# HorizonRobotics/HoloAgent

Measured on AMD Instinct MI355X. Metric: HMSG frames/sec (one scene per GPU: map A1-A2, fusion A3-A5, merge A6, pooling A7, floors A8, rooms by the device watershed N1, room clouds, room embeddings and View nodes A9, objects with the view <-> object test A10 and graph assembly A11, nothing handed in -- plus 1000 coarse-to-fine retrieval qu, higher is better.
Workload: dtype f64 geometry / f32 features

## Files before the change

holoagent_amd/csrc/hmsg_map.hip:

```cpp
#include "hmsg_common.h"

#include <atomic>

#include <algorithm>


__global__ void k_scan_lookback(const unsigned* __restrict__ in, unsigned* __restrict__ out, size_t n,
                                unsigned long long* __restrict__ state, unsigned epoch) {
    __shared__ unsigned wsum[4];
    __shared__ unsigned s_prefix;
    const int tid = threadIdx.x, lane = tid & 63, w = tid >> 6;
    const long long tile = blockIdx.x;
    const size_t base = ((size_t)tile * 256 + tid) * 4;
    unsigned v[4];
    unsigned t = 0;
    for (int i = 0; i < 4; ++i) {
        v[i] = base + i < n ? in[base + i] : 0u;
        t += v[i];
    }
    unsigned incl = t;
    for (int o = 1; o < 64; o <<= 1) {
        unsigned u = __shfl_up(incl, o);
        if (lane >= o) incl += u;
    }
// ... 113 lines not shown
                pix_at(pw, d, f, x, y);
                double w[3];
                if ((unsigned)f == ff && backproject(depth[g], x, y, cam, scale, T, w[0], w[1], w[2])) {
                    for (int a = 0; a < 3; ++a) {
                        mn[a] = w[a] < mn[a] ? w[a] : mn[a];
                        mx[a] = w[a] > mx[a] ? w[a] : mx[a];
                    }
                    cnt++;
                }
            }
        }
    }
    for (int a = 0; a < 3; ++a) {
        mn[a] = wave_min_f64(mn[a]);
        mx[a] = wave_max_f64(mx[a]);
    }
    int c = wave_sum_i32((int)cnt);
    if ((threadIdx.x & 63) == 0) {
        for (int a = 0; a < 3; ++a) {
            atomicMin(&out[a], enc_f64(mn[a]));
            atomicMax(&out[3 + a], enc_f64(mx[a]));
        }
        atomicAdd(npts, (unsigned long long)c);
    }
}

__global__ void k_mark(const unsigned short* __restrict__ depth, const double* __restrict__ pose, CamK cam, float scale,
                       int H, int W, int F, GridGeom g, unsigned long long* __restrict__ bitmap) {
    const size_t HW = (size_t)H * W;
    const size_t total = HW * F;
    for (size_t c0 = (size_t)blockIdx.x * PIX_CHUNK; c0 < total; c0 += (size_t)gridDim.x * PIX_CHUNK) {
        const PixWalk pw = pix_walk(c0, HW, W);
        const unsigned npix = (unsigned)(total - c0 < (size_t)PIX_CHUNK ? total - c0 : (size_t)PIX_CHUNK);
        const unsigned fl = pix_last_frame(pw, npix);
        for (unsigned ff = pw.f0; ff <= fl; ++ff) {
            const double* const T = pose + (size_t)ff * 16;
            for (unsigned d = threadIdx.x; d < npix; d += blockDim.x) {
                const size_t i = c0 + d;
                int f, x, y;
                pix_at(pw, d, f, x, y);
                double wx, wy, wz;
                if ((unsigned)f != ff || !backproject(depth[i], x, y, cam, scale, T, wx, wy, wz)) continue;
                int ix, iy, iz;
                cell_of(g, wx, wy, wz, ix, iy, iz);
                long long lin = lin_of(g, ix, iy, iz);
                unsigned long long bit = 1ull << (lin & 63);
                unsigned long long* wp = bitmap + (lin >> 6);
                if (!(*wp & bit)) atomicOr(wp, bit);
            }
        }
    }
}

struct VoxAcc {
    unsigned long long* sr;
    unsigned long long* sg;
    unsigned long long* sb;
    unsigned* n;
};

#define RUN_CHUNK 4096
__device__ __forceinline__ unsigned pixel_slot(const unsigned short* __restrict__ depth, const double* __restrict__ T ,
                                               const CamK& cam, float scale, size_t i, int x, int y, const GridGeom& g,
                                               const unsigned long long* __restrict__ bitmap, const unsigned* __restrict__ rank) {
    double wx, wy, wz;
    if (!backproject(depth[i], x, y, cam, scale, T, wx, wy, wz)) return 0xffffffffu;
    int ix, iy, iz;
    cell_of(g, wx, wy, wz, ix, iy, iz);
    const long long lin = lin_of(g, ix, iy, iz);
    const unsigned long long word = bitmap[lin >> 6];
    return rank[lin >> 6] + (unsigned)__popcll(word & ((1ull << (lin & 63)) - 1ull));
}

__global__ void __launch_bounds__(256) k_slots(const unsigned short* __restrict__ depth, const unsigned char* __restrict__ rgb,
                                               const double* __restrict__ pose, CamK cam, float scale, int H, int W, int F,
                                               GridGeom g, const unsigned long long* __restrict__ bitmap,
                                               const unsigned* __restrict__ rank, VoxAcc acc, unsigned* __restrict__ slots,
                                               unsigned* __restrict__ chunk_runs) {
    __shared__ unsigned s_runs;
    if (threadIdx.x == 0) s_runs = 0u;
    __syncthreads();
    const size_t HW = (size_t)H * W;
    const size_t total = HW * F;
    const int lane = threadIdx.x & 63;
    unsigned myruns = 0;
    const PixWalk pw = pix_walk((size_t)blockIdx.x * RUN_CHUNK, HW, W);
    const size_t left = total - (size_t)blockIdx.x * RUN_CHUNK;
    const unsigned fl = pix_last_frame(pw, (unsigned)(left < (size_t)RUN_CHUNK ? left : (size_t)RUN_CHUNK));
    for (int it = 0; it < RUN_CHUNK / 256; ++it) {
        const size_t i = (size_t)blockIdx.x * RUN_CHUNK + (size_t)it * 256 + threadIdx.x;
        const bool in_range = i < total;
        unsigned slot = 0xffffffffu;
        unsigned cr = 0, cg = 0, cb = 0, cn = 0;
        int x = 0;
        if (in_range) {
            int f, y;
            pix_at(pw, (unsigned)it * 256u + threadIdx.x, f, x, y);
            for (unsigned ff = pw.f0; ff <= fl; ++ff)
                if ((unsigned)f == ff) slot = pixel_slot(depth, pose + (size_t)ff * 16, cam, scale, i, x, y, g, bitmap, rank);
            slots[i] = slot;
            if (slot != 0xffffffffu) {
                const unsigned char* c = rgb + i * 3;
                cr = c[0];
                cg = c[1];
                cb = c[2];
                cn = 1;
            }
        }
        const unsigned prev = __shfl_up(slot, 1);
        int flag = (lane == 0 || prev != slot || x == 0) ? 1 : 0;
        const int head = flag;
        for (int d = 1; d < 64; d <<= 1) {
            unsigned tr = __shfl_up(cr, d), tg = __shfl_up(cg, d), tb = __shfl_up(cb, d), tn = __shfl_up(cn, d);
            int tf = __shfl_up(flag, d);
            if (lane >= d && !flag) {
                cr += tr; cg += tg; cb += tb; cn += tn;
                flag = tf;
            }
        }
        const int nhead = __shfl_down(head, 1);
        const bool tail = lane == 63 || nhead != 0;
        if (tail && slot != 0xffffffffu) {
            atomicAdd(&acc.sr[slot], (unsigned long long)cr);
            atomicAdd(&acc.sg[slot], (unsigned long long)cg);
            atomicAdd(&acc.sb[slot], (unsigned long long)cb);
            atomicAdd(&acc.n[slot], cn);
            ++myruns;
        }
    }
    myruns = (unsigned)wave_sum_i32((int)myruns);
    if (lane == 0 && myruns) atomicAdd(&s_runs, myruns);
    __syncthreads();
    if (threadIdx.x == 0) chunk_runs[blockIdx.x] = s_runs;
}

__global__ void __launch_bounds__(256) k_emit_runs(const unsigned* __restrict__ slots, size_t total, int W, size_t HW,
                                                   const unsigned* __restrict__ chunk_base, unsigned* __restrict__ keys,
                                                   unsigned long long* __restrict__ vals) {
    __shared__ unsigned s_w[4];
    __shared__ unsigned s_run;
    if (threadIdx.x == 0) s_run = chunk_base[blockIdx.x];
    __syncthreads();
    const int lane = threadIdx.x & 63, w = threadIdx.x >> 6;
    const PixWalk pw = pix_walk((size_t)blockIdx.x * RUN_CHUNK, HW, W);
    for (int it = 0; it < RUN_CHUNK / 256; ++it) {
        const size_t i = (size_t)blockIdx.x * RUN_CHUNK + (size_t)it * 256 + threadIdx.x;
        const bool in_range = i < total;
        const unsigned slot = in_range ? slots[i] : 0xffffffffu;
        int pf = 0, x = 0, py = 0;
        if (in_range) pix_at(pw, (unsigned)it * 256u + threadIdx.x, pf, x, py);
        const unsigned prev = __shfl_up(slot, 1);
        const bool head = lane == 0 || prev != slot || x == 0;
        const unsigned long long heads = __ballot(head);
        const int nhead = __shfl_down(head ? 1 : 0, 1);
        const bool tail = (lane == 63 || nhead != 0) && slot != 0xffffffffu;
        const unsigned long long tails = __ballot(tail);
        if (lane == 0) s_w[w] = (unsigned)__popcll(tails);
        __syncthreads();
        unsigned base = s_run;
        for (int q = 0; q < w; ++q) base += s_w[q];
        if (tail) {
            const unsigned long long below = heads & ((lane == 63) ? ~0ull : ((1ull << (lane + 1)) - 1ull));
            const int start_lane = 63 - __clzll(below);
            const unsigned len = (unsigned)(lane - start_lane + 1);
            const unsigned pos = base + (unsigned)__popcll(tails & ((1ull << lane) - 1ull));
            keys[pos] = slot;
            vals[pos] = ((unsigned long long)(unsigned)pf << 32) | ((unsigned long long)(unsigned)py << 20) |
                        ((unsigned long long)(unsigned)(x - (lane - start_lane)) << 8) | (unsigned long long)len;
        }
        __syncthreads();
        if (threadIdx.x == 0) s_run += s_w[0] + s_w[1] + s_w[2] + s_w[3];
        __syncthreads();
    }
}

template <bool LDS_SUM>
__global__ void __launch_bounds__(256) k_accum_ordered(const unsigned short* __restrict__ depth, const double* __restrict__ pose,
                                                       CamK cam, float scale, int W, size_t HW, long long V,
                                                       const unsigned* __restrict__ off, const unsigned long long* __restrict__ runs,
                                                       const unsigned* __restrict__ cnt, double* __restrict__ pts) {
    __shared__ double s_pt[LDS_SUM ? 4 : 1][LDS_SUM ? 64 * 3 : 1];
    const int lane = threadIdx.x & 63;
    double* const my_pt = s_pt[LDS_SUM ? (threadIdx.x >> 6) : 0];
    const long long v = ((long long)blockIdx.x * blockDim.x + threadIdx.x) >> 6;
    if (v >= V) return;
    double sx = 0.0, sy = 0.0, sz = 0.0;
    const unsigned r0 = off[v], r1 = off[v + 1];
    for (unsigned rb = r0; rb < r1; rb += 64) {
        const unsigned long long myrec = rb + lane < r1 ? runs[rb + lane] : 0ull;
        const int mylen = (int)(myrec & 255ull);
        int incl = mylen;
        for (int o = 1; o < 64; o <<= 1) {
            const int u = __shfl_up(incl, o);
            if (lane >= o) incl += u;
        }
        const int nrun = (int)min(64u, r1 - rb);
        int q0 = 0;
        while (q0 < nrun) {
            const int base = q0 ? __shfl(incl, q0 - 1) : 0;
            const unsigned long long fits = __ballot(lane >= q0 && lane < nrun && incl - base <= 64);
            const int q1 = q0 + __popcll(fits);
            const int npix = __shfl(incl, q1 - 1) - base;
            double wx = 0.0, wy = 0.0, wz = 0.0;
            unsigned long long rec = 0ull;
            int start = 0;
            for (int q = q0; q < q1; ++q) {
                const unsigned long long rq = __shfl(myrec, q);
                const int eq = __shfl(incl, q) - base;
                const int sq = eq - (int)(rq & 255ull);
                if (lane >= sq && lane < eq) {
                    rec = rq;
                    start = sq;
                }
            }
            if (lane < npix) {
                const int f = (int)(rec >> 32);
                const int y = (int)((rec >> 20) & 0xfffull), x0 = (int)((rec >> 8) & 0xfffull);
                const int x = x0 + (lane - start);
                backproject(depth[(size_t)f * HW + (size_t)y * W + x], x, y, cam, scale, pose + (size_t)f * 16, wx, wy, wz);
            }
            if (LDS_SUM) {
                my_pt[lane * 3] = wx;
                my_pt[lane * 3 + 1] = wy;
                my_pt[lane * 3 + 2] = wz;
                __builtin_amdgcn_wave_barrier();
                if (lane < 3)
                    for (int j = 0; j < npix; ++j) sx = __dadd_rn(sx, my_pt[j * 3 + lane]);
                __builtin_amdgcn_wave_barrier();
            } else {
                for (int j = 0; j < npix; ++j) {
                    sx = __dadd_rn(sx, wave_bcast_f64(wx, j));
                    sy = __dadd_rn(sy, wave_bcast_f64(wy, j));
                    sz = __dadd_rn(sz, wave_bcast_f64(wz, j));
                }
            }
            q0 = q1;
        }
    }
    if (LDS_SUM) {
        if (lane < 3) pts[v * 3 + lane] = __ddiv_rn(sx, (double)cnt[v]);
    } else if (lane == 0) {
        const double n = (double)cnt[v];
        pts[v * 3 + 0] = __ddiv_rn(sx, n);
        pts[v * 3 + 1] = __ddiv_rn(sy, n);
        pts[v * 3 + 2] = __ddiv_rn(sz, n);
    }
}

__global__ void k_slot_cells(const unsigned long long* __restrict__ bitmap, const unsigned* __restrict__ rank,
                             GridGeom g, int* __restrict__ cell ) {
    long long w = (long long)blockIdx.x * blockDim.x + threadIdx.x;
    if (w >= g.nwords) return;
    unsigned long long bits = bitmap[w];
    unsigned s = rank[w];
    while (bits) {
        int b = __ffsll(bits) - 1;
        bits &= bits - 1;
        long long lin = w * 64 + b;
        int iz = (int)(lin % g.nzp);
        long long r = lin / g.nzp;
        int iy = (int)(r % g.ny);
        int ix = (int)(r / g.ny);
        cell[(size_t)s * 3 + 0] = ix;
        cell[(size_t)s * 3 + 1] = iy;
        cell[(size_t)s * 3 + 2] = iz;
        ++s;
    }
}

__global__ void k_finalize(VoxAcc acc, long long V, double* __restrict__ cols) {
    long long s = (long long)blockIdx.x * blockDim.x + threadIdx.x;
    if (s >= V) return;
    double n = (double)acc.n[s];
    cols[s * 3 + 0] = ((double)acc.sr[s] / 255.0) / n;
    cols[s * 3 + 1] = ((double)acc.sg[s] / 255.0) / n;
    cols[s * 3 + 2] = ((double)acc.sb[s] / 255.0) / n;
}

__device__ __forceinline__ unsigned long long bits_range(int lo, int hi) {
    if (hi < lo) return 0ull;
    unsigned long long m = (hi >= 63) ? ~0ull : ((1ull << (hi + 1)) - 1ull);
    return m & ~((1ull << lo) - 1ull);
}

__global__ void k_outlier(const double* __restrict__ pts, const int* __restrict__ cell, long long V, GridGeom g,
                          const unsigned long long* __restrict__ bitmap, const unsigned* __restrict__ rank,
                          double radius, int nb_points, unsigned* __restrict__ keep) {
    const int lane = threadIdx.x & 63;
    const long long s = ((long long)blockIdx.x * blockDim.x + threadIdx.x) >> 6;
    if (s >= V) return;
    const double px = pts[s * 3], py = pts[s * 3 + 1], pz = pts[s * 3 + 2];
    const int cx = cell[s * 3], cy = cell[s * 3 + 1];
    const int R = (int)ceil(radius / g.vs) + 1;
    const int side = 2 * R + 1;
    const double r2 = radius * radius;
    const double slack = 1e-7;
    int count = 0;
    for (int c = lane; c < side * side; c += 64) {
        int ix = cx - R + c / side, iy = cy - R + c % side;
        if (ix < 0 || iy < 0 || ix >= g.nx || iy >= g.ny) continue;
        double xlo = g.ox + ix * g.vs, xhi = xlo + g.vs, ylo = g.oy + iy * g.vs, yhi = ylo + g.vs;
        double dxmin = fmax(0.0, fmax(xlo - px, px - xhi)), dxmax = fmax(fabs(px - xlo), fabs(px - xhi));
        double dymin = fmax(0.0, fmax(ylo - py, py - yhi)), dymax = fmax(fabs(py - ylo), fabs(py - yhi));
        dxmin = fmax(0.0, dxmin - slack);
        dymin = fmax(0.0, dymin - slack);
        dxmax += slack;
        dymax += slack;
        double rem_out = r2 - (dxmin * dxmin + dymin * dymin);
        if (rem_out <= 0.0) continue;
        double ho = sqrt(rem_out) + slack;
        int zo0 = (int)floor((pz - ho - g.oz) / g.vs), zo1 = (int)floor((pz + ho - g.oz) / g.vs);
        zo0 = zo0 < 0 ? 0 : zo0;
        zo1 = zo1 >= g.nz ? g.nz - 1 : zo1;
        if (zo1 < zo0) continue;
        double rem_in = r2 - (dxmax * dxmax + dymax * dymax);
        int zi0 = 1, zi1 = 0;
        if (rem_in > 0.0) {
            double hi_ = sqrt(rem_in) - slack;
            if (hi_ > 0.0) {
                zi0 = (int)ceil((pz - hi_ - g.oz) / g.vs);
                zi1 = (int)floor((pz + hi_ - g.oz) / g.vs) - 1;
                zi0 = zi0 < zo0 ? zo0 : zi0;
                zi1 = zi1 > zo1 ? zo1 : zi1;
            }
        }
        long long colw = ((long long)ix * g.ny + iy) * (g.nzp >> 6);
        for (int w = zo0 >> 6; w <= zo1 >> 6; ++w) {
            unsigned long long word = bitmap[colw + w];
            if (!word) continue;
// ... 146 lines not shown
            });
    }
}

void hmsg_build_map(hmsg_ctx* h) {
    const hmsg_config& c = h->cfg;
    hipStream_t s = h->stream;
    HMSG_REQUIRE(h->n_frames > 0, HMSG_ERR_INVALID, "hmsg_finalize_map: no frames added");
    HMSG_REQUIRE(c.voxel_size >= 0.01, HMSG_ERR_UNSUPPORTED,
                 "voxel_size < 0.01: the DBSCAN(0.01,100) of graph.py:352 is no longer a provable no-op");
    const int H = c.height, W = c.width, F = h->n_frames;
    const float scale = (float)c.depth_scale;
    const size_t total = (size_t)H * W * F;
    const unsigned nblk = (unsigned)std::min<size_t>(cdiv(total, 256), 256 * 8);

    DevBuf<unsigned long long> d_b;
    d_b.alloc(8);
    unsigned long long init[8] = {~0ull, ~0ull, ~0ull, 0ull, 0ull, 0ull, 0ull, 0ull};
    HIP_TRY(hipMemcpyAsync(d_b.p, init, sizeof(init), hipMemcpyHostToDevice, s));
    hipLaunchKernelGGL(k_bounds, dim3(nblk), dim3(256), 0, s, (const unsigned short*)h->depth.p,
                       (const double*)h->pose.p, h->cam, scale, H, W, F, d_b.p, d_b.p + 6);
    HMSG_CHECK_LAUNCH();
    unsigned long long hb[8];
    HIP_TRY(hipMemcpyAsync(hb, d_b.p, sizeof(hb), hipMemcpyDeviceToHost, s));
    HIP_TRY(hipStreamSynchronize(s));
    HMSG_REQUIRE(hb[6] > 0, HMSG_ERR_INVALID, "no valid depth pixel in any frame");
    double mn[3], mx[3];
    for (int a = 0; a < 3; ++a) {
        mn[a] = dec_f64(hb[a]);
        mx[a] = dec_f64(hb[3 + a]);
    }
    GridGeom g;
    g.vs = c.voxel_size;
    g.ox = mn[0] - g.vs * 0.5;
    g.oy = mn[1] - g.vs * 0.5;
    g.oz = mn[2] - g.vs * 0.5;
    g.nx = (int)floor((mx[0] - g.ox) / g.vs) + 2;
    g.ny = (int)floor((mx[1] - g.oy) / g.vs) + 2;
    g.nz = (int)floor((mx[2] - g.oz) / g.vs) + 2;
    g.nzp = (g.nz + 63) / 64 * 64;
    g.nwords = (long long)g.nx * g.ny * (g.nzp / 64);
    HMSG_REQUIRE(g.nwords < (1ll << 31), HMSG_ERR_UNSUPPORTED, "scene bounding box too large for the dense occupancy bitmap");
    h->grid = g;

    h->bitmap.alloc((size_t)g.nwords);
    h->rank.alloc((size_t)g.nwords);
    h->bitmap.zero(s);
    hipLaunchKernelGGL(k_mark, dim3(nblk), dim3(256), 0, s, (const unsigned short*)h->depth.p, (const double*)h->pose.p,
                       h->cam, scale, H, W, F, g, h->bitmap.p);
    HMSG_CHECK_LAUNCH();
    unsigned long long V0 = hmsg_bitmap_rank(h->bitmap.p, h->rank.p, (size_t)g.nwords, s, h->scan_tmp);
    h->V0 = (long long)V0;

    DevBuf<unsigned long long> srgb;
    DevBuf<unsigned> sn, slots, chunk_runs;
    srgb.alloc(V0 * 3);
    sn.alloc(V0);
    srgb.zero(s);
    sn.zero(s);
    slots.alloc(total);
    const unsigned nchunks = cdiv(total, RUN_CHUNK);
    chunk_runs.alloc((size_t)nchunks + 1);
    VoxAcc acc{srgb.p, srgb.p + V0, srgb.p + 2 * V0, sn.p};
    {
        ProfScope ps(h->prof, s, "k_slots", (double)total * 9.0 + (double)V0 * 28.0);
        hipLaunchKernelGGL(k_slots, dim3(nchunks), dim3(256), 0, s, (const unsigned short*)h->depth.p,
                           (const unsigned char*)h->rgb.p, (const double*)h->pose.p, h->cam, scale, H, W, F, g,
                           (const unsigned long long*)h->bitmap.p, (const unsigned*)h->rank.p, acc, slots.p, chunk_runs.p);
    }
    HMSG_CHECK_LAUNCH();
    unsigned long long nruns = 0;
    hmsg_scan_u32(chunk_runs.p, chunk_runs.p, (size_t)nchunks, s, h->scan_tmp, &nruns);
    SortBufs sb;
    sb.keys.alloc((size_t)std::max<unsigned long long>(nruns, 1));
    sb.vals.alloc((size_t)std::max<unsigned long long>(nruns, 1));
    HMSG_REQUIRE(W < 4096 && H < 4096, HMSG_ERR_UNSUPPORTED, "image sides must be below 4096 pixels");
    hipLaunchKernelGGL(k_emit_runs, dim3(nchunks), dim3(256), 0, s, (const unsigned*)slots.p, total, W, (size_t)H * W,
                       (const unsigned*)chunk_runs.p, sb.keys.p, sb.vals.p);
    HMSG_CHECK_LAUNCH();
    {
        ProfScope ps(h->prof, s, "sort_runs", (double)nruns * 12.0 * 4.0);
        hmsg_sort_pairs(sb, (size_t)nruns, bits_for(V0), s);
    }
    DevBuf<unsigned> run_off;
    run_off.alloc(V0 + 1);
    hmsg_sort_segment_starts(sb.res_keys, (size_t)nruns, run_off.p, (unsigned)V0, s);
    DevBuf<int> cell;
    cell.alloc(V0 * 3);
    hipLaunchKernelGGL(k_slot_cells, dim3(cdiv((size_t)g.nwords, 256)), dim3(256), 0, s,
                       (const unsigned long long*)h->bitmap.p, (const unsigned*)h->rank.p, g, cell.p);
    HMSG_CHECK_LAUNCH();
    DevBuf<double> pts0, cols0;
    pts0.alloc(V0 * 3);
    cols0.alloc(V0 * 3);
    {
        static const bool lds_sum = getenv("HMSG_DEBUG_ACCUM_WAVES") == nullptr;
        ProfScope ps(h->prof, s, "k_accum_ordered", (double)total * 2.0 + (double)nruns * 8.0 + (double)V0 * 32.0);
        hipLaunchKernelGGL(lds_sum ? k_accum_ordered<true> : k_accum_ordered<false>, dim3(cdiv(V0 * 64, 256)), dim3(256), 0, s,
                           (const unsigned short*)h->depth.p, (const double*)h->pose.p, h->cam, scale, W, (size_t)H * W, (long long)V0,
                           (const unsigned*)run_off.p, (const unsigned long long*)sb.res_vals, (const unsigned*)sn.p, pts0.p);
        HMSG_CHECK_LAUNCH();
        if (getenv("HMSG_DEBUG_ACCUM_STATS")) {
            std::vector<unsigned> hc((size_t)V0);
            HIP_TRY(hipMemcpyAsync(hc.data(), sn.p, (size_t)V0 * 4, hipMemcpyDeviceToHost, s));
            HIP_TRY(hipStreamSynchronize(s));
            std::sort(hc.begin(), hc.end());
            double tot = 0;
            for (unsigned c : hc) tot += c;
            fprintf(stderr, "[hmsg map] voxels %lld  runs %llu  pixels %.0f  max %u  median %u  p99 %u\n", (long long)V0, nruns, tot, hc.back(),
                    hc[hc.size() / 2], hc[(size_t)(hc.size() * 0.99)]);
            for (unsigned th : {512u, 2048u, 8192u, 32768u, 131072u}) {
                double px = 0;
                long long nv = 0;
                for (unsigned c : hc)
                    if (c > th) px += c, ++nv;
                fprintf(stderr, "[hmsg map]   more than %6u pixels: %7lld voxels holding %.3f of the pixels\n", th, nv, px / tot);
            }
        }
    }
    hipLaunchKernelGGL(k_finalize, dim3(cdiv(V0, 256)), dim3(256), 0, s, acc, (long long)V0, cols0.p);
    HMSG_CHECK_LAUNCH();

    DevBuf<unsigned> keep, newidx;
    keep.alloc(V0);
    newidx.alloc(V0);
    hipLaunchKernelGGL(k_outlier, dim3(cdiv(V0 * 64, 256)), dim3(256), 0, s, (const double*)pts0.p, (const int*)cell.p,
                       (long long)V0, g, (const unsigned long long*)h->bitmap.p, (const unsigned*)h->rank.p,
                       c.outlier_radius, c.outlier_nb_points, keep.p);
    HMSG_CHECK_LAUNCH();
    unsigned long long V = 0;
    hmsg_scan_u32(keep.p, newidx.p, V0, s, h->scan_tmp, &V);
    h->V = (long long)V;
    h->pts.alloc(V * 3);
    h->cols.alloc(V * 3);
    hipLaunchKernelGGL(k_compact, dim3(cdiv(V0, 256)), dim3(256), 0, s, (const unsigned*)keep.p, (const unsigned*)newidx.p,
                       (long long)V0, (const double*)pts0.p, (const double*)cols0.p, (const int*)cell.p, g, h->pts.p,
                       h->cols.p, h->bitmap.p);
    HMSG_CHECK_LAUNCH();
    unsigned long long V2 = hmsg_bitmap_rank(h->bitmap.p, h->rank.p, (size_t)g.nwords, s, h->scan_tmp);
    HMSG_REQUIRE(V2 == V, HMSG_ERR_INVALID, "internal: filtered bitmap population mismatch");
    const long long VR = (long long)V0 - (long long)V;
    h->have_cand = false;
    if (VR > 0 && V > 0) {
        h->bitmap_rm.alloc((size_t)g.nwords);
        h->rank_rm.alloc((size_t)g.nwords);
        h->bitmap_rm.zero(s);
        DevBuf<int> rmcell, rend;
        DevBuf<double> ub2;
        DevBuf<unsigned> ccnt, cursor;
        rmcell.alloc((size_t)VR * 3);
        rend.alloc((size_t)VR);
        ub2.alloc((size_t)VR);
        ccnt.alloc((size_t)VR + 1);
        cursor.alloc((size_t)VR);
        ccnt.zero(s);
        cursor.zero(s);
        hipLaunchKernelGGL(k_rm_cells, dim3(cdiv(V0, 256)), dim3(256), 0, s, (const unsigned*)keep.p, (const unsigned*)newidx.p,
                           (long long)V0, (const int*)cell.p, g, rmcell.p, h->bitmap_rm.p);
        HMSG_CHECK_LAUNCH();
        unsigned long long nrm = hmsg_bitmap_rank(h->bitmap_rm.p, h->rank_rm.p, (size_t)g.nwords, s, h->scan_tmp);
        HMSG_REQUIRE((long long)nrm == VR, HMSG_ERR_INVALID, "internal: removed-cell bitmap population mismatch");
        h->cand_off.alloc((size_t)VR + 1);
        {
            ProfScope ps(h->prof, s, "k_cand");
            hipLaunchKernelGGL(k_cand, dim3(cdiv((size_t)VR * 64, 256)), dim3(256), 0, s, 0, (const int*)rmcell.p, VR, g,
                               (const unsigned long long*)h->bitmap.p, (const unsigned*)h->rank.p, (const double*)h->pts.p, ub2.p,
                               rend.p, ccnt.p, (const unsigned*)nullptr, (int*)nullptr, (unsigned*)nullptr);
        }
        HMSG_CHECK_LAUNCH();
        unsigned long long ncand = 0;
        hmsg_scan_u32(ccnt.p, h->cand_off.p, (size_t)VR + 1, s, h->scan_tmp, &ncand);
        h->cand.alloc((size_t)std::max<unsigned long long>(ncand, 1));
        hipLaunchKernelGGL(k_cand, dim3(cdiv((size_t)VR * 64, 256)), dim3(256), 0, s, 1, (const int*)rmcell.p, VR, g,
                           (const unsigned long long*)h->bitmap.p, (const unsigned*)h->rank.p, (const double*)h->pts.p, ub2.p,
// ... 9 lines not shown
```

holoagent_amd/csrc/hmsg_pool.hip:

```cpp
#include "hmsg_boundary.h"
#include "hmsg_cloudops.h"
#include "hmsg_nn.h"
#include "hmsg_dbscan.h"

#include <algorithm>
#include <cmath>

typedef float f32x16 __attribute__((ext_vector_type(16)));

__global__ void k_pool_nn(const double* __restrict__ q, long long N, NNIndex I, double max_dist, int* __restrict__ idx,
                          unsigned* __restrict__ valid, TieList ties) {
    long long i = (long long)blockIdx.x * blockDim.x + threadIdx.x;
    if (i >= N) return;
    double d2 = 0;
    int ntie = 0;
    int v = nn_search(I, q[i * 3], q[i * 3 + 1], q[i * 3 + 2], &d2, &ntie);
    if (ntie > 1) tie_push(ties, i, q[i * 3], q[i * 3 + 1], q[i * 3 + 2]);
    idx[i] = v;
    valid[i] = (v >= 0 && __dsqrt_rn(d2) <= max_dist) ? 1u : 0u;
}

__global__ void k_pool_gather(const int* __restrict__ idx, const unsigned* __restrict__ valid, const unsigned* __restrict__ pos,
                              long long N, const float* __restrict__ feats, int D, float* __restrict__ X, float* __restrict__ Xn) {
    const int lane = threadIdx.x & 63;
// ... 96 lines not shown
            const float a0 = sa[wr * 64 + (lane & 31)][kk], a1 = sa[wr * 64 + 32 + (lane & 31)][kk];
            const float b0 = sb[wc * 64 + (lane & 31)][kk], b1 = sb[wc * 64 + 32 + (lane & 31)][kk];
            acc[0][0] = __builtin_amdgcn_mfma_f32_32x32x2f32(a0, b0, acc[0][0], 0, 0, 0);
            acc[0][1] = __builtin_amdgcn_mfma_f32_32x32x2f32(a0, b1, acc[0][1], 0, 0, 0);
            acc[1][0] = __builtin_amdgcn_mfma_f32_32x32x2f32(a1, b0, acc[1][0], 0, 0, 0);
            acc[1][1] = __builtin_amdgcn_mfma_f32_32x32x2f32(a1, b1, acc[1][1], 0, 0, 0);
        }
        __syncthreads();
    }
    const bool diag_tile = (ti == tj);
    for (int si = 0; si < 2; ++si)
        for (int sj = 0; sj < 2; ++sj) {
            const int rbase = r0 + wr * 64 + si * 32, cbase = c0 + wc * 64 + sj * 32;
            const int col = cbase + (lane & 31);
            unsigned mirror = 0u;
            for (int r = 0; r < 16; ++r) {
                const int rloc = (r & 3) + 8 * (r >> 2) + 4 * (lane >> 5);
                const int row = rbase + rloc;
                float d = __fadd_rn(-acc[si][sj][r], 1.0f);
                d = fminf(fmaxf(d, 0.f), 2.f);
                if (row == col) d = 0.f;
                const bool nb = row < sg.n && col < sg.n && d <= eps;
                mirror |= (nb ? 1u : 0u) << rloc;
                unsigned long long m = __ballot(nb);
                if ((lane & 31) == 0) {
                    unsigned word = (unsigned)(lane ? (m >> 32) : (m & 0xffffffffull));
                    if (row < sg.n && word) {
                        adj[sg.bit_base + (size_t)row * sg.nw + (cbase >> 5)] = word;
                        atomicAdd(&ncount[sg.row_base + row], (unsigned)__popc(word));
                    }
                }
            }
            if (!diag_tile) {
                unsigned other = __shfl_xor(mirror, 32);
                unsigned word = mirror | other;
                if (lane < 32 && col < sg.n && word) {
                    adj[sg.bit_base + (size_t)col * sg.nw + (rbase >> 5)] = word;
                    atomicAdd(&ncount[sg.row_base + col], (unsigned)__popc(word));
                }
            }
        }
}

__global__ void k_pool_init(const unsigned* __restrict__ ncount, long long N, int minpts, int* __restrict__ label,
                            const PoolSeg* __restrict__ segs, const int* __restrict__ seg_of_row, int* __restrict__ seg_first) {
    long long i = (long long)blockIdx.x * blockDim.x + threadIdx.x;
    if (i >= N) return;
    const int k = seg_of_row[i];
    const PoolSeg sg = segs[k];
    const bool is_core = ncount[i] >= (unsigned)minpts;
    label[i] = is_core ? (int)(i - sg.row_base) : -1;
    if (is_core && (int)(i - sg.row_base) < seg_first[k]) atomicMin(&seg_first[k], (int)(i - sg.row_base));
}
__global__ void k_pool_prop(const unsigned* __restrict__ adj, const PoolSeg* __restrict__ segs, const int* __restrict__ seg_of_row,
                            const unsigned* __restrict__ ncount, int minpts, long long N, int* __restrict__ label,
                            int* __restrict__ changed, const int* __restrict__ seg_first, int first_round,
                            const unsigned* __restrict__ list ) {
    const int lane = threadIdx.x & 63;
    long long i = ((long long)blockIdx.x * blockDim.x + threadIdx.x) >> 6;
    if (i >= N) return;
    if (list) i = list[i];
    if (ncount[i] < (unsigned)minpts) return;
    const int k = seg_of_row[i];
    int best = label[i];
    const int lowest = seg_first[k];
    if (best == lowest) return;
    const PoolSeg sg = segs[k];
    const unsigned* row = adj + sg.bit_base + (size_t)(i - sg.row_base) * sg.nw;
    if (first_round) {
        for (int w = lane; w < sg.nw; w += 64) {
            unsigned bits = row[w];
            bool found = false;
            while (bits && !found) {
                const int b = __ffs(bits) - 1;
                bits &= bits - 1;
                const int jr = w * 32 + b;
                if (jr >= best) {
                    found = true;
                } else if (ncount[sg.row_base + jr] >= (unsigned)minpts) {
                    best = jr;
                    found = true;
                }
            }
            if (found) break;
        }
    } else {
        for (int w0 = 0; w0 < sg.nw; w0 += 64) {
            const int w = w0 + lane;
            unsigned bits = w < sg.nw ? row[w] : 0u;
            while (bits && best != lowest) {
                int b = __ffs(bits) - 1;
                bits &= bits - 1;
                long long j = sg.row_base + (long long)w * 32 + b;
                if (ncount[j] >= (unsigned)minpts) {
                    const int lj = label[j];
                    best = lj < best ? lj : best;
                }
            }
            if (__any(best == lowest)) break;
        }
    }
    for (int o = 32; o > 0; o >>= 1) {
        int t = __shfl_xor(best, o);
        best = t < best ? t : best;
    }
    if (lane == 0 && best < label[i]) {
        atomicMin(&label[i], best);
        *changed = 1;
    }
}
__global__ void k_pool_jump(const PoolSeg* __restrict__ segs, const int* __restrict__ seg_of_row, const unsigned* __restrict__ ncount,
                            int minpts, long long N, int* __restrict__ label, const unsigned* __restrict__ list) {
    long long i = (long long)blockIdx.x * blockDim.x + threadIdx.x;
    if (i >= N) return;
    if (list) i = list[i];
    if (ncount[i] < (unsigned)minpts) return;
    const long long base = segs[seg_of_row[i]].row_base;
    int l = label[i];
    for (int hop = 0; hop < 64; ++hop) {
        const int p = label[base + l];
        if (p >= l) break;
        l = p;
    }
    if (l < label[i]) atomicMin(&label[i], l);
}
__global__ void k_pool_list(const PoolSeg* __restrict__ segs, const int* __restrict__ seg_of_row, const unsigned* __restrict__ ncount,
                            int minpts, long long N, const int* __restrict__ label, const int* __restrict__ seg_first,
                            unsigned* __restrict__ list, unsigned* __restrict__ n_list) {
    const long long i = (long long)blockIdx.x * blockDim.x + threadIdx.x;
    const bool open = i < N && ncount[i] >= (unsigned)minpts && label[i] != seg_first[seg_of_row[i]];
    const unsigned long long m = __ballot(open);
    if (!m) return;
    const int lane = threadIdx.x & 63, leader = __ffsll(m) - 1;
    unsigned base = 0;
    if (lane == leader) base = atomicAdd(n_list, (unsigned)__popcll(m));
    base = __shfl(base, leader);
    if (open) list[base + (unsigned)__popcll(m & ((1ull << lane) - 1ull))] = (unsigned)i;
}
__global__ void k_pool_border(const unsigned* __restrict__ adj, const PoolSeg* __restrict__ segs, const int* __restrict__ seg_of_row,
                              const unsigned* __restrict__ ncount, int minpts, long long N, const int* __restrict__ label,
                              int* __restrict__ final_label, unsigned* __restrict__ csize, unsigned* __restrict__ cfirst) {
    const int lane = threadIdx.x & 63;
    const long long i = ((long long)blockIdx.x * blockDim.x + threadIdx.x) >> 6;
    if (i >= N) return;
    const PoolSeg sg = segs[seg_of_row[i]];
    int best;
    if (ncount[i] >= (unsigned)minpts) {
        best = label[i];
    } else {
        best = 0x7fffffff;
        const unsigned* row = adj + sg.bit_base + (size_t)(i - sg.row_base) * sg.nw;
        for (int w = lane; w < sg.nw; w += 64) {
            unsigned bits = row[w];
            while (bits) {
                int b = __ffs(bits) - 1;
                bits &= bits - 1;
                long long j = sg.row_base + (long long)w * 32 + b;
                if (ncount[j] >= (unsigned)minpts) best = label[j] < best ? label[j] : best;
            }
        }
        for (int o = 32; o > 0; o >>= 1) {
            int t = __shfl_xor(best, o);
            best = t < best ? t : best;
        }
        if (best == 0x7fffffff) best = -1;
    }
    if (lane == 0) {
        final_label[i] = best;
        if (best >= 0) {
            atomicAdd(&csize[sg.row_base + best], 1u);
            atomicMin(&cfirst[sg.row_base + best], (unsigned)(i - sg.row_base));
        }
    }
}
__global__ void k_pool_pick(const PoolSeg* __restrict__ segs, const int* __restrict__ seg_of_row, long long N,
                            const unsigned* __restrict__ csize, const unsigned* __restrict__ cfirst,
                            unsigned long long* __restrict__ best) {
// ... 30 lines not shown
    int curl[POOL_MEAN_AHEAD], nxtl[POOL_MEAN_AHEAD];
#pragma unroll
    for (int j = 0; j < POOL_MEAN_AHEAD; ++j) {
        const int rr = min(j, sg.n - 1);
        cur[j] = xb[(size_t)rr * D];
        curl[j] = lb[rr];
    }
    for (int r = 0; r < sg.n; r += POOL_MEAN_AHEAD) {
        if (r + POOL_MEAN_AHEAD < sg.n) {
#pragma unroll
            for (int j = 0; j < POOL_MEAN_AHEAD; ++j) {
                const int rr = min(r + POOL_MEAN_AHEAD + j, sg.n - 1);
                nxt[j] = xb[(size_t)rr * D];
                nxtl[j] = lb[rr];
            }
        }
#pragma unroll
        for (int j = 0; j < POOL_MEAN_AHEAD; ++j) {
            if (r + j < sg.n && (want == -2 || curl[j] == want)) {
                acc = __fadd_rn(acc, cur[j]);
                ++cnt;
            }
        }
#pragma unroll
        for (int j = 0; j < POOL_MEAN_AHEAD; ++j) {
            cur[j] = nxt[j];
            curl[j] = nxtl[j];
        }
    }
    o[d] = cnt > 1 ? __fdiv_rn(acc, (float)cnt) : acc;
}

__global__ void k_pool_gather_u32(const unsigned* __restrict__ src, const long long* __restrict__ idx, int n,
                                  unsigned* __restrict__ dst) {
    int t = blockIdx.x * blockDim.x + threadIdx.x;
    if (t < n) dst[t] = src[idx[t]];
}
__global__ void k_seg_rows(const PoolSeg* __restrict__ segs, int* __restrict__ seg_of_row) {
    const PoolSeg sg = segs[blockIdx.y];
    for (int i = blockIdx.x * blockDim.x + threadIdx.x; i < sg.n; i += gridDim.x * blockDim.x) seg_of_row[sg.row_base + i] = blockIdx.y;
}

void pool_cluster(hipStream_t s, const PoolSeg* d_ps, long long R, int minpts, const unsigned* adj, const unsigned* ncount,
                  const int* seg_of_row, int* label, int* seg_first, int* d_changed, int* flabel, unsigned* csize, unsigned* cfirst,
                  unsigned long long* best, DbgLaps* laps) {
    hipLaunchKernelGGL(k_pool_init, dim3(cdiv((size_t)R, 256)), dim3(256), 0, s, ncount, (long long)R,
                       minpts, label, d_ps, seg_of_row, seg_first);
    HMSG_CHECK_LAUNCH();
    DevBuf<unsigned> open_list;
    open_list.alloc((size_t)std::max<long long>(R, 1) + 1);
    const unsigned* d_list = nullptr;
    unsigned n_open = 0;
    static const bool list_wanted = getenv("HMSG_DEBUG_POOL_ALL_ROWS") == nullptr;
    for (int it = 0; it < 100000; ++it) {
        HIP_TRY(hipMemsetAsync(d_changed, 0, 4, s));
        const size_t rows = d_list ? (size_t)n_open : (size_t)R;
        for (int rep = 0; rep < (it == 0 ? 2 : 1) && rows; ++rep) {
            hipLaunchKernelGGL(k_pool_prop, dim3(cdiv(rows * 64, 256)), dim3(256), 0, s, adj,
                               d_ps, seg_of_row, ncount,
                               minpts, (long long)rows, label, d_changed, seg_first, (it == 0 && rep == 0) ? 1 : 0, d_list);
            hipLaunchKernelGGL(k_pool_jump, dim3(cdiv(rows, 256)), dim3(256), 0, s, d_ps,
                               seg_of_row, ncount, minpts, (long long)rows, label, d_list);
        }
        HMSG_CHECK_LAUNCH();
        if (it == 0 && list_wanted) {
            HIP_TRY(hipMemsetAsync(open_list.p, 0, 4, s));
            hipLaunchKernelGGL(k_pool_list, dim3(cdiv((size_t)R, 256)), dim3(256), 0, s, d_ps, seg_of_row,
                               ncount, minpts, (long long)R, label, seg_first,
                               open_list.p + 1, open_list.p);
            HMSG_CHECK_LAUNCH();
            HIP_TRY(hipMemcpyAsync(&n_open, open_list.p, 4, hipMemcpyDeviceToHost, s));
        }
        int ch = 0;
        HIP_TRY(hipMemcpyAsync(&ch, d_changed, 4, hipMemcpyDeviceToHost, s));
        HIP_TRY(hipStreamSynchronize(s));
        if (it == 0 && list_wanted) d_list = open_list.p + 1;
        if (!ch) break;
    }
    if (laps) laps->lap("label propagation");
    hipLaunchKernelGGL(k_pool_border, dim3(cdiv((size_t)R * 64, 256)), dim3(256), 0, s, adj,
                       d_ps, seg_of_row, ncount, minpts,
                       (long long)R, label, flabel, csize, cfirst);
    hipLaunchKernelGGL(k_pool_pick, dim3(cdiv((size_t)R, 256)), dim3(256), 0, s, d_ps,
                       seg_of_row, (long long)R, csize, cfirst, best);
    HMSG_CHECK_LAUNCH();
}

void pool_launch_gram_f32(hipStream_t s, const float* Xn, int D, const PoolSeg* d_ps, int K, long long tiles, float eps, unsigned* adj,
                          unsigned* ncount) {
    hipLaunchKernelGGL(k_pool_gram, dim3((unsigned)tiles), dim3(256), 0, s, Xn, D, d_ps, K, eps, adj, ncount);
    HMSG_CHECK_LAUNCH();
}
void pool_launch_seg_rows(hipStream_t s, const PoolSeg* d_ps, int K, int maxn, int* seg_of_row) {
    hipLaunchKernelGGL(k_seg_rows, dim3(std::max(1u, std::min(cdiv(maxn, 256), 256u)), K), dim3(256), 0, s, d_ps, seg_of_row);
    HMSG_CHECK_LAUNCH();
}
void pool_launch_mean_f32(hipStream_t s, const float* X, int D, const PoolSeg* d_ps, int K, const int* flabel, const unsigned* csize,
                          const unsigned* cfirst, const unsigned long long* best, float* out) {
    hipLaunchKernelGGL(k_pool_mean, dim3(cdiv(D, 64), K), dim3(64), 0, s, X, D, d_ps, K, flabel, csize, cfirst, best, out);
    HMSG_CHECK_LAUNCH();
}

static void pool_rows(hipStream_t s, DevBuf<unsigned>& scan_tmp, Prof* prof, DbgLaps& laps, const int* idx, const unsigned* valid,
                      long long P, const std::vector<int>& dn, const float* feats, int D, double eps, int minpts, float* out) {
    const int K = (int)dn.size();
    DevBuf<unsigned> pos;
    pos.alloc((size_t)std::max<long long>(P, 1));
    unsigned long long R = 0;
    if (P) hmsg_scan_u32(valid, pos.p, (size_t)P, s, scan_tmp, &R);
    std::vector<long long> pstart(K + 1, 0);
    for (int k = 0; k < K; ++k) pstart[k + 1] = pstart[k] + dn[k];
    std::vector<unsigned> hpos(K + 1, (unsigned)R);
    {
        DevBuf<long long> d_i;
        DevBuf<unsigned> d_o;
        std::vector<long long> q;
        std::vector<int> which;
        for (int k = 0; k < K; ++k)
            if (pstart[k] < P) {
                q.push_back(pstart[k]);
                which.push_back(k);
            }
        if (!q.empty()) {
            std::vector<unsigned> tmp(q.size());
            d_i.alloc(q.size());
// ... 175 lines not shown
```

Before: 2737.

## Fold colour sums into ordered accumulation and list-drive second pooling round

Removes the per-pixel RGB segmented scan and the four global atomics per run from k_slots. Colour sums now come from the run records inside k_accum_ordered, which also drops the separate finalize kernel and the colour and count buffers. In pooling, the second first-iteration round now runs after the open-row list is built and reads the list length on the device with grid-stride loops, so it processes only open rows. The label neighbour scan also batches eight loads before reducing. The cost is extra rgb reads and registers in the accumulation kernel and a capped grid for the list-driven round.

```diff
diff --git a/holoagent_amd/csrc/hmsg_map.hip b/holoagent_amd/csrc/hmsg_map.hip
--- a/holoagent_amd/csrc/hmsg_map.hip
+++ b/holoagent_amd/csrc/hmsg_map.hip
@@ -189,13 +189,6 @@
     }
 }
 
-struct VoxAcc {
-    unsigned long long* sr;
-    unsigned long long* sg;
-    unsigned long long* sb;
-    unsigned* n;
-};
-
 #define RUN_CHUNK 4096
 __device__ __forceinline__ unsigned pixel_slot(const unsigned short* __restrict__ depth, const double* __restrict__ T ,
                                                const CamK& cam, float scale, size_t i, int x, int y, const GridGeom& g,
@@ -209,11 +202,24 @@
     return rank[lin >> 6] + (unsigned)__popcll(word & ((1ull << (lin & 63)) - 1ull));
 }
 
-__global__ void __launch_bounds__(256) k_slots(const unsigned short* __restrict__ depth, const unsigned char* __restrict__ rgb,
-                                               const double* __restrict__ pose, CamK cam, float scale, int H, int W, int F,
-                                               GridGeom g, const unsigned long long* __restrict__ bitmap,
-                                               const unsigned* __restrict__ rank, VoxAcc acc, unsigned* __restrict__ slots,
-                                               unsigned* __restrict__ chunk_runs) {
+struct RunEdges {
+    unsigned long long heads, tails;
+    bool tail;
+};
+__device__ __forceinline__ RunEdges run_edges(unsigned slot, int x, int lane) {
+    const unsigned prev = __shfl_up(slot, 1);
+    const bool head = lane == 0 || prev != slot || x == 0;
+    RunEdges e;
+    e.heads = __ballot(head);
+    e.tail = (lane == 63 || ((e.heads >> (lane + 1)) & 1ull)) && slot != 0xffffffffu;
+    e.tails = __ballot(e.tail);
+    return e;
+}
+
+__global__ void __launch_bounds__(256) k_slots(const unsigned short* __restrict__ depth, const double* __restrict__ pose, CamK cam,
+                                               float scale, int H, int W, int F, GridGeom g,
+                                               const unsigned long long* __restrict__ bitmap, const unsigned* __restrict__ rank,
+                                               unsigned* __restrict__ slots, unsigned* __restrict__ chunk_runs) {
     __shared__ unsigned s_runs;
     if (threadIdx.x == 0) s_runs = 0u;
     __syncthreads();
@@ -226,46 +232,17 @@
     const unsigned fl = pix_last_frame(pw, (unsigned)(left < (size_t)RUN_CHUNK ? left : (size_t)RUN_CHUNK));
     for (int it = 0; it < RUN_CHUNK / 256; ++it) {
         const size_t i = (size_t)blockIdx.x * RUN_CHUNK + (size_t)it * 256 + threadIdx.x;
-        const bool in_range = i < total;
         unsigned slot = 0xffffffffu;
-        unsigned cr = 0, cg = 0, cb = 0, cn = 0;
         int x = 0;
-        if (in_range) {
+        if (i < total) {
             int f, y;
             pix_at(pw, (unsigned)it * 256u + threadIdx.x, f, x, y);
             for (unsigned ff = pw.f0; ff <= fl; ++ff)
                 if ((unsigned)f == ff) slot = pixel_slot(depth, pose + (size_t)ff * 16, cam, scale, i, x, y, g, bitmap, rank);
             slots[i] = slot;
-            if (slot != 0xffffffffu) {
-                const unsigned char* c = rgb + i * 3;
-                cr = c[0];
-                cg = c[1];
-                cb = c[2];
-                cn = 1;
-            }
-        }
-        const unsigned prev = __shfl_up(slot, 1);
-        int flag = (lane == 0 || prev != slot || x == 0) ? 1 : 0;
-        const int head = flag;
-        for (int d = 1; d < 64; d <<= 1) {
-            unsigned tr = __shfl_up(cr, d), tg = __shfl_up(cg, d), tb = __shfl_up(cb, d), tn = __shfl_up(cn, d);
-            int tf = __shfl_up(flag, d);
-            if (lane >= d && !flag) {
-                cr += tr; cg += tg; cb += tb; cn += tn;
-                flag = tf;
-            }
-        }
-        const int nhead = __shfl_down(head, 1);
-        const bool tail = lane == 63 || nhead != 0;
-        if (tail && slot != 0xffffffffu) {
-            atomicAdd(&acc.sr[slot], (unsigned long long)cr);
-            atomicAdd(&acc.sg[slot], (unsigned long long)cg);
-            atomicAdd(&acc.sb[slot], (unsigned long long)cb);
-            atomicAdd(&acc.n[slot], cn);
-            ++myruns;
-        }
-    }
-    myruns = (unsigned)wave_sum_i32((int)myruns);
+        }
+        myruns += (unsigned)__popcll(run_edges(slot, x, lane).tails);
+    }
     if (lane == 0 && myruns) atomicAdd(&s_runs, myruns);
     __syncthreads();
     if (threadIdx.x == 0) chunk_runs[blockIdx.x] = s_runs;
@@ -286,12 +263,9 @@
         const unsigned slot = in_range ? slots[i] : 0xffffffffu;
         int pf = 0, x = 0, py = 0;
         if (in_range) pix_at(pw, (unsigned)it * 256u + threadIdx.x, pf, x, py);
-        const unsigned prev = __shfl_up(slot, 1);
-        const bool head = lane == 0 || prev != slot || x == 0;
-        const unsigned long long heads = __ballot(head);
-        const int nhead = __shfl_down(head ? 1 : 0, 1);
-        const bool tail = (lane == 63 || nhead != 0) && slot != 0xffffffffu;
-        const unsigned long long tails = __ballot(tail);
+        const RunEdges e = run_edges(slot, x, lane);
+        const unsigned long long heads = e.heads, tails = e.tails;
+        const bool tail = e.tail;
         if (lane == 0) s_w[w] = (unsigned)__popcll(tails);
         __syncthreads();
         unsigned base = s_run;
@@ -313,15 +287,17 @@
 
 template <bool LDS_SUM>
 __global__ void __launch_bounds__(256) k_accum_ordered(const unsigned short* __restrict__ depth, const double* __restrict__ pose,
-                                                       CamK cam, float scale, int W, size_t HW, long long V,
-                                                       const unsigned* __restrict__ off, const unsigned long long* __restrict__ runs,
-                                                       const unsigned* __restrict__ cnt, double* __restrict__ pts) {
+                                                       const unsigned char* __restrict__ rgb, CamK cam, float scale, int W, size_t HW,
+                                                       long long V, const unsigned* __restrict__ off,
+                                                       const unsigned long long* __restrict__ runs, double* __restrict__ pts,
+                                                       double* __restrict__ cols) {
     __shared__ double s_pt[LDS_SUM ? 4 : 1][LDS_SUM ? 64 * 3 : 1];
     const int lane = threadIdx.x & 63;
     double* const my_pt = s_pt[LDS_SUM ? (threadIdx.x >> 6) : 0];
     const long long v = ((long long)blockIdx.x * blockDim.x + threadIdx.x) >> 6;
     if (v >= V) return;
     double sx = 0.0, sy = 0.0, sz = 0.0;
+    unsigned long long cr = 0ull, cg = 0ull, cb = 0ull, npx = 0ull;
     const unsigned r0 = off[v], r1 = off[v + 1];
     for (unsigned rb = r0; rb < r1; rb += 64) {
         const unsigned long long myrec = rb + lane < r1 ? runs[rb + lane] : 0ull;
@@ -354,8 +330,14 @@
                 const int f = (int)(rec >> 32);
                 const int y = (int)((rec >> 20) & 0xfffull), x0 = (int)((rec >> 8) & 0xfffull);
                 const int x = x0 + (lane - start);
-                backproject(depth[(size_t)f * HW + (size_t)y * W + x], x, y, cam, scale, pose + (size_t)f * 16, wx, wy, wz);
-            }
+                const size_t i = (size_t)f * HW + (size_t)y * W + x;
+                backproject(depth[i], x, y, cam, scale, pose + (size_t)f * 16, wx, wy, wz);
+                const unsigned char* const c = rgb + i * 3;
+                cr += c[0];
+                cg += c[1];
+                cb += c[2];
+            }
+            npx += (unsigned long long)npix;
             if (LDS_SUM) {
                 my_pt[lane * 3] = wx;
                 my_pt[lane * 3 + 1] = wy;
@@ -374,14 +356,20 @@
             q0 = q1;
         }
     }
+    for (int o = 32; o > 0; o >>= 1) {
+        cr += __shfl_xor(cr, o);
+        cg += __shfl_xor(cg, o);
+        cb += __shfl_xor(cb, o);
+    }
+    const double n = (double)npx;
     if (LDS_SUM) {
-        if (lane < 3) pts[v * 3 + lane] = __ddiv_rn(sx, (double)cnt[v]);
+        if (lane < 3) pts[v * 3 + lane] = __ddiv_rn(sx, n);
     } else if (lane == 0) {
-        const double n = (double)cnt[v];
         pts[v * 3 + 0] = __ddiv_rn(sx, n);
         pts[v * 3 + 1] = __ddiv_rn(sy, n);
         pts[v * 3 + 2] = __ddiv_rn(sz, n);
     }
+    if (lane < 3) cols[v * 3 + lane] = ((double)(lane == 0 ? cr : lane == 1 ? cg : cb) / 255.0) / n;
 }
 
 __global__ void k_slot_cells(const unsigned long long* __restrict__ bitmap, const unsigned* __restrict__ rank,
@@ -403,15 +391,6 @@
         cell[(size_t)s * 3 + 2] = iz;
         ++s;
     }
-}
-
-__global__ void k_finalize(VoxAcc acc, long long V, double* __restrict__ cols) {
-    long long s = (long long)blockIdx.x * blockDim.x + threadIdx.x;
-    if (s >= V) return;
-    double n = (double)acc.n[s];
-    cols[s * 3 + 0] = ((double)acc.sr[s] / 255.0) / n;
-    cols[s * 3 + 1] = ((double)acc.sg[s] / 255.0) / n;
-    cols[s * 3 + 2] = ((double)acc.sb[s] / 255.0) / n;
 }
 
 __device__ __forceinline__ unsigned long long bits_range(int lo, int hi) {
@@ -664,21 +643,15 @@
     unsigned long long V0 = hmsg_bitmap_rank(h->bitmap.p, h->rank.p, (size_t)g.nwords, s, h->scan_tmp);
     h->V0 = (long long)V0;
 
-    DevBuf<unsigned long long> srgb;
-    DevBuf<unsigned> sn, slots, chunk_runs;
-    srgb.alloc(V0 * 3);
-    sn.alloc(V0);
-    srgb.zero(s);
-    sn.zero(s);
+    DevBuf<unsigned> slots, chunk_runs;
     slots.alloc(total);
     const unsigned nchunks = cdiv(total, RUN_CHUNK);
     chunk_runs.alloc((size_t)nchunks + 1);
-    VoxAcc acc{srgb.p, srgb.p + V0, srgb.p + 2 * V0, sn.p};
     {
-        ProfScope ps(h->prof, s, "k_slots", (double)total * 9.0 + (double)V0 * 28.0);
-        hipLaunchKernelGGL(k_slots, dim3(nchunks), dim3(256), 0, s, (const unsigned short*)h->depth.p,
-                           (const unsigned char*)h->rgb.p, (const double*)h->pose.p, h->cam, scale, H, W, F, g,
-                           (const unsigned long long*)h->bitmap.p, (const unsigned*)h->rank.p, acc, slots.p, chunk_runs.p);
+        ProfScope ps(h->prof, s, "k_slots", (double)total * 6.0);
+        hipLaunchKernelGGL(k_slots, dim3(nchunks), dim3(256), 0, s, (const unsigned short*)h->depth.p, (const double*)h->pose.p,
+                           h->cam, scale, H, W, F, g, (const unsigned long long*)h->bitmap.p, (const unsigned*)h->rank.p, slots.p,
+                           chunk_runs.p);
     }
     HMSG_CHECK_LAUNCH();
     unsigned long long nruns = 0;
@@ -707,15 +680,23 @@
     cols0.alloc(V0 * 3);
     {
         static const bool lds_sum = getenv("HMSG_DEBUG_ACCUM_WAVES") == nullptr;
-        ProfScope ps(h->prof, s, "k_accum_ordered", (double)total * 2.0 + (double)nruns * 8.0 + (double)V0 * 32.0);
+        ProfScope ps(h->prof, s, "k_accum_ordered", (double)total * 5.0 + (double)nruns * 8.0 + (double)V0 * 52.0);
         hipLaunchKernelGGL(lds_sum ? k_accum_ordered<true> : k_accum_ordered<false>, dim3(cdiv(V0 * 64, 256)), dim3(256), 0, s,
-                           (const unsigned short*)h->depth.p, (const double*)h->pose.p, h->cam, scale, W, (size_t)H * W, (long long)V0,
-                           (const unsigned*)run_off.p, (const unsigned long long*)sb.res_vals, (const unsigned*)sn.p, pts0.p);
+                           (const unsigned short*)h->depth.p, (const double*)h->pose.p, (const unsigned char*)h->rgb.p, h->cam, scale, W,
+                           (size_t)H * W, (long long)V0, (const unsigned*)run_off.p, (const unsigned long long*)sb.res_vals, pts0.p,
+                           cols0.p);
         HMSG_CHECK_LAUNCH();
         if (getenv("HMSG_DEBUG_ACCUM_STATS")) {
-            std::vector<unsigned> hc((size_t)V0);
-            HIP_TRY(hipMemcpyAsync(hc.data(), sn.p, (size_t)V0 * 4, hipMemcpyDeviceToHost, s));
+            std::vector<unsigned> ho((size_t)V0 + 1), hc((size_t)V0);
+            std::vector<unsigned long long> hr((size_t)nruns);
+            HIP_TRY(hipMemcpyAsync(ho.data(), run_off.p, ((size_t)V0 + 1) * 4, hipMemcpyDeviceToHost, s));
+            HIP_TRY(hipMemcpyAsync(hr.data(), sb.res_vals, (size_t)nruns * 8, hipMemcpyDeviceToHost, s));
             HIP_TRY(hipStreamSynchronize(s));
+            for (size_t v = 0; v < (size_t)V0; ++v) {
+                unsigned n = 0;
+                for (unsigned r = ho[v]; r < ho[v + 1]; ++r) n += (unsigned)(hr[r] & 255ull);
+                hc[v] = n;
+            }
             std::sort(hc.begin(), hc.end());
             double tot = 0;
             for (unsigned c : hc) tot += c;
@@ -730,8 +711,6 @@
             }
         }
     }
-    hipLaunchKernelGGL(k_finalize, dim3(cdiv(V0, 256)), dim3(256), 0, s, acc, (long long)V0, cols0.p);
-    HMSG_CHECK_LAUNCH();
 
     DevBuf<unsigned> keep, newidx;
     keep.alloc(V0);
diff --git a/holoagent_amd/csrc/hmsg_pool.hip b/holoagent_amd/csrc/hmsg_pool.hip
--- a/holoagent_amd/csrc/hmsg_pool.hip
+++ b/holoagent_amd/csrc/hmsg_pool.hip
@@ -172,14 +172,10 @@
     label[i] = is_core ? (int)(i - sg.row_base) : -1;
     if (is_core && (int)(i - sg.row_base) < seg_first[k]) atomicMin(&seg_first[k], (int)(i - sg.row_base));
 }
-__global__ void k_pool_prop(const unsigned* __restrict__ adj, const PoolSeg* __restrict__ segs, const int* __restrict__ seg_of_row,
-                            const unsigned* __restrict__ ncount, int minpts, long long N, int* __restrict__ label,
-                            int* __restrict__ changed, const int* __restrict__ seg_first, int first_round,
-                            const unsigned* __restrict__ list ) {
-    const int lane = threadIdx.x & 63;
-    long long i = ((long long)blockIdx.x * blockDim.x + threadIdx.x) >> 6;
-    if (i >= N) return;
-    if (list) i = list[i];
+__device__ __forceinline__ void pool_prop_row(const unsigned* __restrict__ adj, const PoolSeg* __restrict__ segs,
+                                              const int* __restrict__ seg_of_row, const unsigned* __restrict__ ncount, int minpts,
+                                              long long i, int* __restrict__ label, int* __restrict__ changed,
+                                              const int* __restrict__ seg_first, int first_round, int lane) {
     if (ncount[i] < (unsigned)minpts) return;
     const int k = seg_of_row[i];
     int best = label[i];
@@ -209,13 +205,18 @@
             const int w = w0 + lane;
             unsigned bits = w < sg.nw ? row[w] : 0u;
             while (bits && best != lowest) {
-                int b = __ffs(bits) - 1;
-                bits &= bits - 1;
-                long long j = sg.row_base + (long long)w * 32 + b;
-                if (ncount[j] >= (unsigned)minpts) {
-                    const int lj = label[j];
-                    best = lj < best ? lj : best;
+                int lj[8];
+#pragma unroll
+                for (int q = 0; q < 8; ++q) {
+                    lj[q] = -1;
+                    if (bits) {
+                        const int b = __ffs(bits) - 1;
+                        bits &= bits - 1;
+                        lj[q] = label[sg.row_base + (long long)w * 32 + b];
+                    }
                 }
+#pragma unroll
+                for (int q = 0; q < 8; ++q) best = (unsigned)lj[q] < (unsigned)best ? lj[q] : best;
             }
             if (__any(best == lowest)) break;
         }
@@ -229,20 +230,33 @@
         *changed = 1;
     }
 }
+__global__ void k_pool_prop(const unsigned* __restrict__ adj, const PoolSeg* __restrict__ segs, const int* __restrict__ seg_of_row,
+                            const unsigned* __restrict__ ncount, int minpts, long long N, int* __restrict__ label,
+                            int* __restrict__ changed, const int* __restrict__ seg_first, int first_round,
+                            const unsigned* __restrict__ list ,
+                            const unsigned* __restrict__ n_list ) {
+    const int lane = threadIdx.x & 63;
+    const long long nwaves = ((long long)gridDim.x * blockDim.x) >> 6;
+    if (n_list) N = (long long)*n_list;
+    for (long long e = ((long long)blockIdx.x * blockDim.x + threadIdx.x) >> 6; e < N; e += nwaves)
+        pool_prop_row(adj, segs, seg_of_row, ncount, minpts, list ? (long long)list[e] : e, label, changed, seg_first, first_round, lane);
+}
 __global__ void k_pool_jump(const PoolSeg* __restrict__ segs, const int* __restrict__ seg_of_row, const unsigned* __restrict__ ncount,
-                            int minpts, long long N, int* __restrict__ label, const unsigned* __restrict__ list) {
-    long long i = (long long)blockIdx.x * blockDim.x + threadIdx.x;
-    if (i >= N) return;
-    if (list) i = list[i];
-    if (ncount[i] < (unsigned)minpts) return;
-    const long long base = segs[seg_of_row[i]].row_base;
-    int l = label[i];
-    for (int hop = 0; hop < 64; ++hop) {
-        const int p = label[base + l];
-        if (p >= l) break;
-        l = p;
-    }
-    if (l < label[i]) atomicMin(&label[i], l);
+                            int minpts, long long N, int* __restrict__ label, const unsigned* __restrict__ list,
+                            const unsigned* __restrict__ n_list ) {
+    if (n_list) N = (long long)*n_list;
+    for (long long e = (long long)blockIdx.x * blockDim.x + threadIdx.x; e < N; e += (long long)gridDim.x * blockDim.x) {
+        const long long i = list ? (long long)list[e] : e;
+        if (ncount[i] < (unsigned)minpts) continue;
+        const long long base = segs[seg_of_row[i]].row_base;
+        int l = label[i];
+        for (int hop = 0; hop < 64; ++hop) {
+            const int p = label[base + l];
+            if (p >= l) break;
+            l = p;
+        }
+        if (l < label[i]) atomicMin(&label[i], l);
+    }
 }
 __global__ void k_pool_list(const PoolSeg* __restrict__ segs, const int* __restrict__ seg_of_row, const unsigned* __restrict__ ncount,
                             int minpts, long long N, const int* __restrict__ label, const int* __restrict__ seg_first,
@@ -379,25 +393,30 @@
     const unsigned* d_list = nullptr;
     unsigned n_open = 0;
     static const bool list_wanted = getenv("HMSG_DEBUG_POOL_ALL_ROWS") == nullptr;
+    const auto round = [&](size_t rows, unsigned wave_blocks, int first_round, const unsigned* list, const unsigned* n_list) {
+        hipLaunchKernelGGL(k_pool_prop, dim3(wave_blocks), dim3(256), 0, s, adj, d_ps, seg_of_row, ncount, minpts, (long long)rows,
+                           label, d_changed, seg_first, first_round, list, n_list);
+        hipLaunchKernelGGL(k_pool_jump, dim3(n_list ? wave_blocks : cdiv(rows, 256)), dim3(256), 0, s, d_ps, seg_of_row, ncount, minpts,
+                           (long long)rows, label, list, n_list);
+    };
     for (int it = 0; it < 100000; ++it) {
         HIP_TRY(hipMemsetAsync(d_changed, 0, 4, s));
-        const size_t rows = d_list ? (size_t)n_open : (size_t)R;
-        for (int rep = 0; rep < (it == 0 ? 2 : 1) && rows; ++rep) {
-            hipLaunchKernelGGL(k_pool_prop, dim3(cdiv(rows * 64, 256)), dim3(256), 0, s, adj,
-                               d_ps, seg_of_row, ncount,
-                               minpts, (long long)rows, label, d_changed, seg_first, (it == 0 && rep == 0) ? 1 : 0, d_list);
-            hipLaunchKernelGGL(k_pool_jump, dim3(cdiv(rows, 256)), dim3(256), 0, s, d_ps,
-                               seg_of_row, ncount, minpts, (long long)rows, label, d_list);
+        if (it == 0 && R > 0) {
+            round((size_t)R, cdiv((size_t)R * 64, 256), 1, nullptr, nullptr);
+            if (list_wanted) {
+                HIP_TRY(hipMemsetAsync(open_list.p, 0, 4, s));
+                hipLaunchKernelGGL(k_pool_list, dim3(cdiv((size_t)R, 256)), dim3(256), 0, s, d_ps, seg_of_row,
+                                   ncount, minpts, (long long)R, label, seg_first,
+                                   open_list.p + 1, open_list.p);
+                round((size_t)R, std::min(cdiv((size_t)R * 64, 256), 32768u), 0, open_list.p + 1, open_list.p);
+                HIP_TRY(hipMemcpyAsync(&n_open, open_list.p, 4, hipMemcpyDeviceToHost, s));
+            } else {
+                round((size_t)R, cdiv((size_t)R * 64, 256), 0, nullptr, nullptr);
+            }
+        } else if (const size_t rows = d_list ? (size_t)n_open : (size_t)R) {
+            round(rows, cdiv(rows * 64, 256), 0, d_list, nullptr);
         }
         HMSG_CHECK_LAUNCH();
-        if (it == 0 && list_wanted) {
-            HIP_TRY(hipMemsetAsync(open_list.p, 0, 4, s));
-            hipLaunchKernelGGL(k_pool_list, dim3(cdiv((size_t)R, 256)), dim3(256), 0, s, d_ps, seg_of_row,
-                               ncount, minpts, (long long)R, label, seg_first,
-                               open_list.p + 1, open_list.p);
-            HMSG_CHECK_LAUNCH();
-            HIP_TRY(hipMemcpyAsync(&n_open, open_list.p, 4, hipMemcpyDeviceToHost, s));
-        }
         int ch = 0;
         HIP_TRY(hipMemcpyAsync(&ch, d_changed, 4, hipMemcpyDeviceToHost, s));
         HIP_TRY(hipStreamSynchronize(s));
```

After: 2789, median of 6. 1.02x the previous value.
